# alibaba/TorchEasyRec

Measured on NVIDIA H100. Metric: samples/sec (DLRM-Criteo synth, train step fwd+bwd+optimizer), higher is better.
Workload: dtype f32

## Files before the change

### torcheasyrec_b200/csrc/tzk_interact_wide.cu

```cuda
#include <stdint.h>
#include <stdio.h>
#include <stdlib.h>

#ifdef TZK_CPU_SHIM
#include "cuda_cpu_shim.h"
#include "sm90_cpu_emu.h"
#include "sm90_wgmma_emu.h"
typedef void* tzk_stream_t;
#define TZK_REQUIRE(cond, ...) do { if (!(cond)) return 1; } while (0)
#define TZK_CHECK_LAUNCH(name) do {} while (0)
#else
#include <cuda.h>
#include "tzk_common.cuh"
#define TZK_DYN_SMEM(type, name) extern __shared__ __align__(1024) type name[]
#define TZK_UNPAREN(...) __VA_ARGS__
#define TZK_LAUNCH(kernel, grid, block, smem, stream, ...) TZK_UNPAREN kernel<<<grid, block, smem, stream>>>(__VA_ARGS__)
#endif

namespace {
#ifndef TZK_CPU_SHIM
#include "tzk_sm90_ptx.h"
#endif
#include "tzk_tma.h"
#include "tzk_wgmma.cuh"
namespace tzk_itc {
__device__ __forceinline__ uint32_t cvt_tf32(float x) { return tf32_bits(x); }
__device__ __forceinline__ void mma_tf32(float (&c)[4], const uint32_t (&a)[4], const uint32_t (&b)[2]) { ::mma_tf32(c, a, b); }
}
#include "tzk_interact_tc.cuh"

__device__ __forceinline__ float4 load_l2(const float* p) {
#ifdef TZK_CPU_SHIM
  return *reinterpret_cast<const float4*>(p);
#else
  return __ldcg(reinterpret_cast<const float4*>(p));
#endif
}

constexpr int FB_M = 64;
constexpr int FB_THREADS = 512;
constexpr int FB_WARPS = FB_THREADS / 32;
constexpr int FB_CHUNKS = (tzk_itc::kRow + 31) / 32;
constexpr int FB_PAIR_CHUNKS = tzk_itc::kInter / 32;
constexpr int FB_BOX = 32 * 128;
constexpr int FB_STAGE = 4 * FB_BOX;
constexpr int FB_STAGES = 3;
constexpr int FB_LDP = 360;
constexpr int FB_P_OFF = FB_STAGES * FB_STAGE;
constexpr int FB_S_OFF = FB_P_OFF + FB_M * FB_LDP * 4;
constexpr int FB_IJ_OFF = FB_S_OFF + FB_WARPS * 32 * tzk_itc::kSS * 4;
constexpr int FB_BAR_OFF = FB_IJ_OFF + tzk_itc::kInter * 2;
constexpr int FB_SMEM = FB_BAR_OFF + FB_STAGES * 8;

struct FbParams {
  const float* dz; int64_t ld_dz;
  const float* dense; int64_t ld_dense;
  const float* sparse; int64_t ld_sparse;
  float* d_dense; int64_t ld_ddense;
  float* d_sparse; int64_t ld_dsparse;
  int64_t M;
};

__global__ void __launch_bounds__(FB_THREADS, 1)
interact_wide_bwd_kernel(const __grid_constant__ CUtensorMap map_whi, const __grid_constant__ CUtensorMap map_wlo,
                         FbParams p) {
  TZK_DYN_SMEM(uint8_t, smem);
  float* P = reinterpret_cast<float*>(smem + FB_P_OFF);
  uint64_t* full = reinterpret_cast<uint64_t*>(smem + FB_BAR_OFF);
  const int warp = threadIdx.x >> 5, lane = threadIdx.x & 31, g = lane >> 2, t = lane & 3;
  const int64_t m0 = (int64_t)blockIdx.x * FB_M;

  if (threadIdx.x == 0) {
    for (int s = 0; s < FB_STAGES; ++s) mbar_init(full + s, 1);
    fence_mbarrier_init();
  }
  float* S = reinterpret_cast<float*>(smem + FB_S_OFF) + warp * (32 * tzk_itc::kSS);
  unsigned short* pair_ij = reinterpret_cast<unsigned short*>(smem + FB_IJ_OFF);
  tzk_itc::init_pair_ij(pair_ij);
  for (int i = lane; i < 32 * tzk_itc::kSS; i += 32) S[i] = 0.f;
  __syncthreads();
  auto col_chunk = [](int c) { return (c + FB_PAIR_CHUNKS) % FB_CHUNKS; };
  auto load = [&](int c) {
    uint8_t* sb = smem + (c % FB_STAGES) * FB_STAGE;
    uint64_t* bar = full + c % FB_STAGES;
    const int n0 = col_chunk(c) * 32;
    mbar_expect_tx(bar, FB_STAGE);
    tma_load_2d(sb, &map_whi, bar, 0, n0);
    tma_load_2d(sb + FB_BOX, &map_whi, bar, 32, n0);
    tma_load_2d(sb + 2 * FB_BOX, &map_wlo, bar, 0, n0);
    tma_load_2d(sb + 3 * FB_BOX, &map_wlo, bar, 32, n0);
  };
  if (threadIdx.x == 0)
    for (int c = 0; c < FB_STAGES; ++c) load(c);

  const int wm = warp & 3, wn = warp >> 2;
  const int r = wm * 16 + g;
  uint32_t ah[8][4], al[8][4];
#pragma unroll
  for (int kk = 0; kk < 8; ++kk) {
    const int k0 = kk * 8 + t, k1 = k0 + 4;
    const int64_t ra = m0 + r, rb = ra + 8;
    const float a[4] = {ra < p.M ? __ldg(p.dz + ra * p.ld_dz + k0) : 0.f, rb < p.M ? __ldg(p.dz + rb * p.ld_dz + k0) : 0.f,
                        ra < p.M ? __ldg(p.dz + ra * p.ld_dz + k1) : 0.f, rb < p.M ? __ldg(p.dz + rb * p.ld_dz + k1) : 0.f};
#pragma unroll
    for (int i = 0; i < 4; ++i) {
      ah[kk][i] = tf32_bits(a[i]);
      al[kk][i] = tf32_bits(a[i] - __uint_as_float(ah[kk][i]));
    }
  }
  const int n = wn * 8 + g;
  for (int c = 0; c < FB_CHUNKS; ++c) {
    const int s = c % FB_STAGES;
    mbar_wait(full + s, (uint32_t)(c / FB_STAGES) & 1u);
    const uint32_t* whi = reinterpret_cast<const uint32_t*>(smem + s * FB_STAGE);
    const uint32_t* wlo = whi + 2 * FB_BOX / 4;
    float acc[4] = {0.f, 0.f, 0.f, 0.f};
#pragma unroll
    for (int kk = 0; kk < 8; ++kk) {
      const uint32_t* bh_box = whi + (kk >> 2) * (FB_BOX / 4);
      const uint32_t* bl_box = wlo + (kk >> 2) * (FB_BOX / 4);
      const int k0 = (kk & 3) * 8 + t, k1 = k0 + 4;
      const uint32_t bh[2] = {bh_box[swz(n, k0)], bh_box[swz(n, k1)]};
      const uint32_t bl[2] = {bl_box[swz(n, k0)], bl_box[swz(n, k1)]};
      float part[4] = {0.f, 0.f, 0.f, 0.f};
      mma_tf32(part, al[kk], bh);
      mma_tf32(part, ah[kk], bl);
      mma_tf32(part, ah[kk], bh);
#pragma unroll
      for (int q = 0; q < 4; ++q) acc[q] += part[q];
    }
    const int col = col_chunk(c) * 32 + wn * 8 + 2 * t;
    if (col < tzk_itc::kInter) {
      *reinterpret_cast<float2*>(P + r * FB_LDP + col) = make_float2(acc[0], acc[1]);
      *reinterpret_cast<float2*>(P + (r + 8) * FB_LDP + col) = make_float2(acc[2], acc[3]);
    } else if (col < tzk_itc::kRow) {
      const int e = col - tzk_itc::kInter;
#pragma unroll
      for (int h = 0; h < 2; ++h) {
        const int64_t row = m0 + r + 8 * h;
        if (row >= p.M) continue;
        float* dst = e < tzk_itc::kD ? p.d_dense + row * p.ld_ddense + e : p.d_sparse + row * p.ld_dsparse + (e - tzk_itc::kD);
        *reinterpret_cast<float2*>(dst) = make_float2(acc[2 * h], acc[2 * h + 1]);
      }
    }
    __syncthreads();
    if (threadIdx.x == 0 && c + FB_STAGES < FB_CHUNKS) load(c + FB_STAGES);
  }

  for (int i = warp; i < FB_M; i += FB_WARPS) {
    const int64_t b = m0 + i;
    if (b >= p.M) break;
    float* dd = p.d_dense + b * p.ld_ddense;
    float* ds = p.d_sparse + b * p.ld_dsparse;
    float4 pass[4];
#pragma unroll
    for (int q = 0; q < 4; ++q) {
      const int row = g + 8 * q;
      pass[q] = row == 0 ? load_l2(dd + 4 * t)
              : row < tzk_itc::kN ? load_l2(ds + (row - 1) * tzk_itc::kD + 4 * t)
              : make_float4(0.f, 0.f, 0.f, 0.f);
    }
    tzk_itc::bwd_sample(P + i * FB_LDP, p.dense + b * p.ld_dense, p.sparse + b * p.ld_sparse, pass, pair_ij, S, dd, ds,
                        lane);
  }
}

constexpr int FF_M = 128;
constexpr int FF_THREADS = 256;
constexpr int FF_WARPS = FF_THREADS / 32;
constexpr int FF_X_BYTES = FF_M * 128;
constexpr int FF_W_BYTES = 64 * 128;
constexpr int FF_STAGE = FF_X_BYTES + 2 * FF_W_BYTES;
constexpr int FF_STAGES = 3;
constexpr int FF_E_OFF = FF_STAGES * FF_STAGE;
constexpr int FF_BAR_OFF = FF_E_OFF + FF_X_BYTES;
constexpr int FF_SMEM = FF_BAR_OFF + FF_STAGES * 8;
static_assert(FF_WARPS * tzk_itc::kInter * 4 <= FF_X_BYTES, "staging rows overflow their region");
constexpr int FF_SPARSE0 = tzk_itc::kInter + tzk_itc::kD;

struct FfParams {
  const float* dense; int64_t ld_dense;
  const float* sparse; int64_t ld_sparse;
  float* pairs; int64_t ld_pairs;
  const float* bias;
  float* y; int64_t ld_y;
  int64_t M;
};

__device__ __forceinline__ void fence_proxy_async() {
#ifndef TZK_CPU_SHIM
  asm volatile("fence.proxy.async;" ::: "memory");
#endif
}

__global__ void __launch_bounds__(FF_THREADS, 2)
interact_wide_fwd_kernel(const __grid_constant__ CUtensorMap map_pairs, const __grid_constant__ CUtensorMap map_dense,
                         const __grid_constant__ CUtensorMap map_sparse, const __grid_constant__ CUtensorMap map_whi, const __grid_constant__ CUtensorMap map_wlo,
                         FfParams p) {
  TZK_DYN_SMEM(uint8_t, smem);
  uint64_t* full = reinterpret_cast<uint64_t*>(smem + FF_BAR_OFF);
  const int warp = threadIdx.x >> 5, lane = threadIdx.x & 31, g = lane >> 2, t = lane & 3;
  const int64_t m0 = (int64_t)blockIdx.x * FF_M;
  const int64_t m_end = p.M - m0 < FF_M ? p.M : m0 + FF_M;

  if (threadIdx.x == 0) {
    for (int s = 0; s < FF_STAGES; ++s) mbar_init(full + s, 1);
    fence_mbarrier_init();
  }
  {
    float* O = reinterpret_cast<float*>(smem + FF_E_OFF) + warp * tzk_itc::kInter;
    if (lane == 0) O[tzk_itc::kP] = 0.f;
    int rowbase[4];
    tzk_itc::pair_rowbase(g, rowbase);
    int64_t b = m0 + warp;
    float4 x[4];
    if (b < m_end) {
#pragma unroll
      for (int j = 0; j < 4; ++j) x[j] = tzk_itc::load_x4(p.dense + b * p.ld_dense, p.sparse + b * p.ld_sparse, g + 8 * j, 4 * t);
    }
    for (; b < m_end; b += FF_WARPS) {
      float4 xn[4];
      const int64_t bn = b + FF_WARPS;
      if (bn < m_end) {
#pragma unroll
        for (int j = 0; j < 4; ++j)
          xn[j] = tzk_itc::load_x4(p.dense + bn * p.ld_dense, p.sparse + bn * p.ld_sparse, g + 8 * j, 4 * t);
      }
      tzk_itc::fwd_sample(x, rowbase, O, p.pairs + b * p.ld_pairs, lane);
      if (bn < m_end) {
#pragma unroll
        for (int j = 0; j < 4; ++j) x[j] = xn[j];
      }
    }
  }
  fence_proxy_async();
  __syncthreads();

  auto load = [&](int c) {
    uint8_t* sb = smem + (c % FF_STAGES) * FF_STAGE;
    uint64_t* bar = full + c % FF_STAGES;
    mbar_expect_tx(bar, c == FB_PAIR_CHUNKS ? FF_STAGE + FF_X_BYTES : FF_STAGE);
    if (c < FB_PAIR_CHUNKS) {
      tma_load_2d(sb, &map_pairs, bar, 32 * c, (int)m0);
    } else if (c == FB_PAIR_CHUNKS) {
      tma_load_2d(sb, &map_dense, bar, 0, (int)m0);
      tma_load_2d(smem + FF_E_OFF, &map_sparse, bar, 0, (int)m0);
    } else {
      tma_load_2d(sb, &map_sparse, bar, 32 * c - FF_SPARSE0, (int)m0);
    }
    tma_load_2d(sb + FF_X_BYTES, &map_whi, bar, 32 * c, 0);
    tma_load_2d(sb + FF_X_BYTES + FF_W_BYTES, &map_wlo, bar, 32 * c, 0);
  };
  if (threadIdx.x == 0)
    for (int c = 0; c < FF_STAGES; ++c) load(c);

  const int r = warp * 16 + g;
  float acc[32], part[32];
#pragma unroll
  for (int i = 0; i < 32; ++i) acc[i] = 0.f;
  for (int c = 0; c < FB_CHUNKS; ++c) {
    const int s = c % FF_STAGES;
    mbar_wait(full + s, (uint32_t)(c / FF_STAGES) & 1u);
    const float* xs = reinterpret_cast<const float*>(smem + s * FF_STAGE);
    const uint8_t* whi = smem + s * FF_STAGE + FF_X_BYTES;
    const uint8_t* wlo = whi + FF_W_BYTES;
#pragma unroll
    for (int ks = 0; ks < 4; ++ks) {
      const int k0 = ks * 8 + t, k1 = k0 + 4;
      const bool sp = ks >= 2 && c == FB_PAIR_CHUNKS;
      const float* as = sp ? reinterpret_cast<const float*>(smem + FF_E_OFF) : xs;
      const int x16 = sp ? 16 : 0;
      const float a[4] = {as[swz(r, k0) ^ x16], as[swz(r + 8, k0) ^ x16], as[swz(r, k1) ^ x16], as[swz(r + 8, k1) ^ x16]};
      uint32_t ah[4], al[4];
#pragma unroll
      for (int i = 0; i < 4; ++i) {
        ah[i] = tf32_bits(a[i]);
        al[i] = tf32_bits(a[i] - __uint_as_float(ah[i]));
      }
      wgmma_fence();
      wgmma_3xtf32<64>(part, ah, al, wgmma_desc(whi, ks), wgmma_desc(wlo, ks));
      wgmma_commit();
      wgmma_wait<0>();
#pragma unroll
      for (int i = 0; i < 32; ++i) {
        wgmma_reg_fence(part[i]);
        acc[i] += part[i];
      }
    }
    __syncthreads();
    if (threadIdx.x == 0 && c + FF_STAGES < FB_CHUNKS) load(c + FF_STAGES);
  }
#pragma unroll
  for (int nt = 0; nt < 8; ++nt) {
    const int col = nt * 8 + 2 * t;
    const float b0 = p.bias ? __ldg(p.bias + col) : 0.f, b1 = p.bias ? __ldg(p.bias + col + 1) : 0.f;
#pragma unroll
    for (int h = 0; h < 2; ++h) {
      const int64_t row = m0 + r + 8 * h;
      if (row >= p.M) continue;
      float2 o = make_float2(acc[4 * nt + 2 * h] + b0, acc[4 * nt + 2 * h + 1] + b1);
      o.x = fmaxf(o.x, 0.f);
      o.y = fmaxf(o.y, 0.f);
      *reinterpret_cast<float2*>(p.y + row * p.ld_y + col) = o;
    }
  }
}

__global__ void split_w_kernel(const float* __restrict__ w, int64_t ld_w, int K, float* __restrict__ hi,
                               float* __restrict__ lo) {
  const int i = blockIdx.x * blockDim.x + threadIdx.x;
  if (i < K * 64) {
    const float v = w[(int64_t)(i / K) * ld_w + i % K];
    const float h = tf32_rna(v);
    hi[i] = h;
    lo[i] = tf32_rna(v - h);
  }
}

#include "tzk_wgrad3x.cuh"

constexpr int WW_ZT = 64 * 128;

__global__ void __launch_bounds__(WG_THREADS, 2)
interact_wide_wgrad_kernel(const __grid_constant__ CUtensorMap map_x0, const __grid_constant__ CUtensorMap map_x1,
                           const __grid_constant__ CUtensorMap map_x2, const __grid_constant__ CUtensorMap map_dz,
                           WgParams p) {
  TZK_DYN_SMEM(uint8_t, smem);
  uint8_t* zt = smem + WG_STAGES * WG_STAGE;
  uint64_t* full = reinterpret_cast<uint64_t*>(zt + 2 * WW_ZT);
  int* boxes = reinterpret_cast<int*>(full + WG_STAGES);

  const int warp = threadIdx.x >> 5, lane = threadIdx.x & 31, g = lane >> 2, t = lane & 3;
  const int jt = blockIdx.x % p.k_tiles;
  const int64_t slab = blockIdx.x / p.k_tiles;
  const int64_t row0 = slab * p.slab_rows;
  const int64_t rows = (p.M - row0 < p.slab_rows) ? p.M - row0 : p.slab_rows;
  const int num_c = (int)((rows + WG_ROWS - 1) / WG_ROWS);

  if (threadIdx.x == 0) {
    for (int s = 0; s < WG_STAGES; ++s) mbar_init(full + s, 1);
    fence_mbarrier_init();
    for (int b = 0; b < 4; ++b) {
      const int box = jt * 4 + b, s = wg_source(p.src, box);
      boxes[b] = s;
      boxes[4 + b] = wg_pick(p.src.col0, s) + 32 * (box - wg_pick(p.src.first, s));
    }
  }
  __syncthreads();
  auto load = [&](int c) {
    uint8_t* sb = smem + (c % WG_STAGES) * WG_STAGE;
    uint64_t* bar = full + c % WG_STAGES;
    const int r = (int)(row0 + (int64_t)c * WG_ROWS);
    mbar_expect_tx(bar, WG_A + WG_B);
#pragma unroll 1
    for (int b = 0; b < 4; ++b) {
      const int s = *reinterpret_cast<volatile int*>(boxes + b), col = *reinterpret_cast<volatile int*>(boxes + 4 + b);
      tma_load_2d(sb + b * WG_BOX, s == 0 ? &map_x0 : s == 1 ? &map_x1 : &map_x2, bar, col, r);
    }
#pragma unroll
    for (int b = 0; b < 2; ++b) tma_load_2d(sb + WG_A + b * WG_BOX, &map_dz, bar, b * 32, r);
  };
  if (threadIdx.x == 0)
    for (int c = 0; c < WG_STAGES && c < num_c; ++c) load(c);

  const int xc = (warp >> 2) * 64 + (warp & 3) * 16 + g;
  const int tn = threadIdx.x & 63, tq = threadIdx.x >> 6;
  uint32_t* zhi = reinterpret_cast<uint32_t*>(zt);
  uint32_t* zlo = zhi + WW_ZT / 4;
  float acc[32], part[32];
#pragma unroll
  for (int i = 0; i < 32; ++i) acc[i] = 0.f;
  for (int c = 0; c < num_c; ++c) {
    const int s = c % WG_STAGES;
    mbar_wait(full + s, (uint32_t)(c / WG_STAGES) & 1u);
    const float* xs = reinterpret_cast<const float*>(smem + s * WG_STAGE);
    const float* zs = reinterpret_cast<const float*>(smem + s * WG_STAGE + WG_A);
    auto at = [](const float* base, int m, int col) { return base[(col >> 5) * (WG_BOX / 4) + swz(m, col & 31)]; };
#pragma unroll
    for (int h = 0; h < 2; ++h) {
      const int m = 4 * tq + 16 * h;
      float hi[4], lo[4];
#pragma unroll
      for (int j = 0; j < 4; ++j) {
        const float v = at(zs, m + j, tn);
        hi[j] = tf32_rna(v);
        lo[j] = tf32_rna(v - hi[j]);
      }
      *reinterpret_cast<float4*>(zhi + swz(tn, m)) = make_float4(hi[0], hi[1], hi[2], hi[3]);
      *reinterpret_cast<float4*>(zlo + swz(tn, m)) = make_float4(lo[0], lo[1], lo[2], lo[3]);
    }
    fence_proxy_async();
    __syncthreads();
#pragma unroll
    for (int ks = 0; ks < WG_ROWS / 8; ++ks) {
      const int m = ks * 8 + t;
      const float a[4] = {at(xs, m, xc), at(xs, m, xc + 8), at(xs, m + 4, xc), at(xs, m + 4, xc + 8)};
      uint32_t ah[4], al[4];
#pragma unroll
      for (int i = 0; i < 4; ++i) {
        ah[i] = tf32_bits(a[i]);
        al[i] = tf32_bits(a[i] - __uint_as_float(ah[i]));
      }
      wgmma_fence();
      wgmma_tf32<64>(part, ah, wgmma_desc(zlo, ks), false);
      wgmma_tf32<64>(part, al, wgmma_desc(zhi, ks), true);
      wgmma_tf32<64>(part, ah, wgmma_desc(zhi, ks), true);
      wgmma_commit();
      wgmma_wait<0>();
#pragma unroll
      for (int i = 0; i < 32; ++i) {
        wgmma_reg_fence(part[i]);
        acc[i] += part[i];
      }
    }
    __syncthreads();
    if (threadIdx.x == 0 && c + WG_STAGES < num_c) load(c + WG_STAGES);
  }
  float* out = p.partial + ((int64_t)slab * p.k_tiles + jt) * 128 * 64;
#pragma unroll
  for (int i = 0; i < 8; ++i)
#pragma unroll
    for (int h = 0; h < 2; ++h)
      *reinterpret_cast<float2*>(out + (int64_t)(xc + 8 * h) * 64 + 8 * i + 2 * t) =
          make_float2(acc[4 * i + 2 * h], acc[4 * i + 2 * h + 1]);
}

__global__ void split_wt_kernel(const float* __restrict__ w, int64_t ld_w, int K, float* __restrict__ hi,
                                float* __restrict__ lo) {
  const int i = blockIdx.x * blockDim.x + threadIdx.x;
  if (i < K * 64) {
    const int k = i >> 6, o = i & 63;
    const float v = w[(int64_t)o * ld_w + k];
    const float h = tf32_rna(v);
    hi[i] = h;
    lo[i] = tf32_rna(v - h);
  }
}

}

extern "C" int tzk_interact_wide_bwd(const float* dz, int64_t ld_dz, const float* w, int64_t ld_w, const float* dense,
                                     int64_t ld_dense, const float* sparse, int64_t ld_sparse, int64_t M, float* d_dense,
                                     int64_t ld_ddense, float* d_sparse, int64_t ld_dsparse, float* wt_hi, float* wt_lo,
                                     tzk_stream_t stream) {
  TZK_REQUIRE(M > 0, "interact_wide_bwd: M must be positive");
  TZK_REQUIRE(ld_w >= tzk_itc::kRow, "interact_wide_bwd: w needs %d columns", tzk_itc::kRow);
  const int64_t lds[] = {ld_dz, ld_w, ld_dense, ld_sparse, ld_ddense, ld_dsparse};
  for (int64_t ld : lds) TZK_REQUIRE(ld % 4 == 0, "interact_wide_bwd: row strides must be multiples of 4 floats");
  const void* ptrs[] = {dz, w, dense, sparse, d_dense, d_sparse, wt_hi, wt_lo};
  for (const void* q : ptrs)
    TZK_REQUIRE(q && reinterpret_cast<uintptr_t>(q) % 16 == 0, "interact_wide_bwd: NULL or not 16-B aligned pointer");
  cudaStream_t st = reinterpret_cast<cudaStream_t>(stream);
  TZK_LAUNCH((split_wt_kernel), (tzk_itc::kRow * 64 + 255) / 256, 256, 0, st, w, ld_w, tzk_itc::kRow, wt_hi, wt_lo);
  CUtensorMap mh, ml;
  TZK_REQUIRE(!make_map(&mh, wt_hi, tzk_itc::kRow, 64, 64, 32) && !make_map(&ml, wt_lo, tzk_itc::kRow, 64, 64, 32),
              "interact_wide_bwd: tensor-map encoding failed");
  FbParams p;
  p.dz = dz; p.ld_dz = ld_dz; p.dense = dense; p.ld_dense = ld_dense; p.sparse = sparse; p.ld_sparse = ld_sparse;
  p.d_dense = d_dense; p.ld_ddense = ld_ddense; p.d_sparse = d_sparse; p.ld_dsparse = ld_dsparse; p.M = M;
#ifndef TZK_CPU_SHIM
  static bool configured = false;
  if (!configured) {
    cudaFuncSetAttribute(interact_wide_bwd_kernel, cudaFuncAttributeMaxDynamicSharedMemorySize, FB_SMEM);
    configured = true;
  }
#endif
  TZK_LAUNCH((interact_wide_bwd_kernel), (unsigned)((M + FB_M - 1) / FB_M), FB_THREADS, FB_SMEM, st, mh, ml, p);
  TZK_CHECK_LAUNCH("interact_wide_bwd_kernel");
  return 0;
}

extern "C" int tzk_interact_wide_fwd(const float* dense, int64_t ld_dense, const float* sparse, int64_t ld_sparse,
                                     const float* w, int64_t ld_w, const float* bias, int64_t M, float* y, int64_t ld_y,
                                     float* pairs, int64_t ld_pairs, float* w_hi, float* w_lo, tzk_stream_t stream) {
  TZK_REQUIRE(M > 0, "interact_wide_fwd: M must be positive");
  TZK_REQUIRE(ld_w >= tzk_itc::kRow && ld_y >= 64 && ld_pairs >= tzk_itc::kInter && ld_dense >= tzk_itc::kD &&
              ld_sparse >= tzk_itc::kRow - FF_SPARSE0, "interact_wide_fwd: row stride shorter than the row");
  const int64_t lds[] = {ld_dense, ld_sparse, ld_w, ld_y, ld_pairs};
  for (int64_t ld : lds) TZK_REQUIRE(ld % 4 == 0, "interact_wide_fwd: row strides must be multiples of 4 floats");
  const void* ptrs[] = {dense, sparse, w, y, pairs, w_hi, w_lo};
  for (const void* q : ptrs)
    TZK_REQUIRE(q && reinterpret_cast<uintptr_t>(q) % 16 == 0, "interact_wide_fwd: NULL or not 16-B aligned pointer");
  cudaStream_t st = reinterpret_cast<cudaStream_t>(stream);
  TZK_LAUNCH((split_w_kernel), (tzk_itc::kRow * 64 + 255) / 256, 256, 0, st, w, ld_w, tzk_itc::kRow, w_hi, w_lo);
  CUtensorMap mp, md, ms, mh, ml;
  TZK_REQUIRE(!make_map(&mp, pairs, M, tzk_itc::kInter, ld_pairs, FF_M) &&
              !make_map(&md, dense, M, tzk_itc::kD, ld_dense, FF_M) &&
              !make_map(&ms, sparse, M, tzk_itc::kRow - FF_SPARSE0, ld_sparse, FF_M) &&
              !make_map(&mh, w_hi, 64, tzk_itc::kRow, tzk_itc::kRow, 64) &&
              !make_map(&ml, w_lo, 64, tzk_itc::kRow, tzk_itc::kRow, 64), "interact_wide_fwd: tensor-map encoding failed");
  FfParams p;
  p.dense = dense; p.ld_dense = ld_dense; p.sparse = sparse; p.ld_sparse = ld_sparse; p.pairs = pairs;
  p.ld_pairs = ld_pairs; p.bias = bias; p.y = y; p.ld_y = ld_y; p.M = M;
#ifndef TZK_CPU_SHIM
  static bool configured = false;
  if (!configured) {
    cudaFuncSetAttribute(interact_wide_fwd_kernel, cudaFuncAttributeMaxDynamicSharedMemorySize, FF_SMEM);
    configured = true;
  }
#endif
  TZK_LAUNCH((interact_wide_fwd_kernel), (unsigned)((M + FF_M - 1) / FF_M), FF_THREADS, FF_SMEM, st, mp, md, ms, mh, ml, p);
  TZK_CHECK_LAUNCH("interact_wide_fwd_kernel");
  return 0;
}

extern "C" int tzk_interact_wide_wgrad(const float* dz, int64_t ld_dz, const float* pairs, int64_t ld_pairs,
                                       const float* dense, int64_t ld_dense, const float* sparse, int64_t ld_sparse,
                                       int64_t M, int32_t slabs, float* partial, float* dw, int64_t ld_dw,
                                       tzk_stream_t stream) {
  TZK_REQUIRE(M > 0 && slabs > 0, "interact_wide_wgrad: M and slabs must be positive");
  TZK_REQUIRE(ld_dw >= tzk_itc::kRow, "interact_wide_wgrad: dw needs %d columns", tzk_itc::kRow);
  const int64_t lds[] = {ld_dz, ld_pairs, ld_dense, ld_sparse};
  for (int64_t ld : lds) TZK_REQUIRE(ld % 4 == 0, "interact_wide_wgrad: row strides must be multiples of 4 floats");
  const void* ptrs[] = {dz, pairs, dense, sparse, partial, dw};
  for (const void* q : ptrs)
    TZK_REQUIRE(q && reinterpret_cast<uintptr_t>(q) % 16 == 0, "interact_wide_wgrad: NULL or not 16-B aligned pointer");
  CUtensorMap mx[WG_SRC], mz;
  TZK_REQUIRE(!make_map(&mx[0], pairs, M, tzk_itc::kInter, ld_pairs, WG_ROWS) &&
              !make_map(&mx[1], sparse, M, tzk_itc::kRow - FF_SPARSE0, ld_sparse, WG_ROWS) &&
              !make_map(&mx[2], dense, M, tzk_itc::kD, ld_dense, WG_ROWS) &&
              !make_map(&mz, dz, M, 64, ld_dz, WG_ROWS), "interact_wide_wgrad: tensor-map encoding failed");
  const WgSources src = {{0, FB_PAIR_CHUNKS, FB_CHUNKS - 1, FB_CHUNKS}, {0, 0, 0}, {0, FF_SPARSE0, tzk_itc::kInter},
                         {tzk_itc::kInter, tzk_itc::kRow - FF_SPARSE0, tzk_itc::kD}};
  TZK_REQUIRE(wgrad3x_launch<interact_wide_wgrad_kernel>(mx, mz, src, M, slabs, partial, dw, ld_dw,
                                                         reinterpret_cast<cudaStream_t>(stream), 2 * WW_ZT) == 0,
              "interact_wide_wgrad: launch failed");
  return 0;
}
```

### torcheasyrec_b200/csrc/tzk_sm90_ptx.h

```cpp

__device__ __forceinline__ uint32_t smem_u32(const void* p) { return (uint32_t)__cvta_generic_to_shared(p); }

__device__ __forceinline__ void mbar_init(uint64_t* bar, uint32_t count) {
  asm volatile("mbarrier.init.shared::cta.b64 [%0], %1;" ::"r"(smem_u32(bar)), "r"(count));
}
__device__ __forceinline__ void mbar_expect_tx(uint64_t* bar, uint32_t bytes) {
  asm volatile("mbarrier.arrive.expect_tx.shared::cta.b64 _, [%0], %1;" ::"r"(smem_u32(bar)), "r"(bytes) : "memory");
}
__device__ __forceinline__ void mbar_wait(uint64_t* bar, uint32_t parity) {
  asm volatile(
      "{\n\t.reg .pred p;\n\t"
      "WAIT_LOOP:\n\t"
      "mbarrier.try_wait.parity.shared::cta.b64 p, [%0], %1;\n\t"
      "@p bra DONE;\n\t"
      "bra WAIT_LOOP;\n\t"
      "DONE:\n\t}" ::"r"(smem_u32(bar)), "r"(parity)
      : "memory");
}
__device__ __forceinline__ void fence_mbarrier_init() { asm volatile("fence.mbarrier_init.release.cluster;" ::: "memory"); }

__device__ __forceinline__ void tma_load_2d(void* dst, const CUtensorMap* map, uint64_t* bar, int c0, int c1) {
  asm volatile(
      "cp.async.bulk.tensor.2d.shared::cluster.global.mbarrier::complete_tx::bytes [%0], [%1, {%3, %4}], [%2];"
      ::"r"(smem_u32(dst)), "l"(map), "r"(smem_u32(bar)), "r"(c0), "r"(c1)
      : "memory");
}

__device__ __forceinline__ uint32_t tf32_bits(float x) {
  uint32_t r;
  asm("cvt.rna.tf32.f32 %0, %1;" : "=r"(r) : "f"(x));
  return r;
}
__device__ __forceinline__ float tf32_rna(float x) { return __uint_as_float(tf32_bits(x)); }
__device__ __forceinline__ void mma_tf32(float (&c)[4], const uint32_t (&a)[4], const uint32_t (&b)[2]) {
  asm volatile("mma.sync.aligned.m16n8k8.row.col.f32.tf32.tf32.f32 {%0,%1,%2,%3}, {%4,%5,%6,%7}, {%8,%9}, {%0,%1,%2,%3};"
               : "+f"(c[0]), "+f"(c[1]), "+f"(c[2]), "+f"(c[3])
               : "r"(a[0]), "r"(a[1]), "r"(a[2]), "r"(a[3]), "r"(b[0]), "r"(b[1]));
}
```

### torcheasyrec_b200/csrc/tzk_wgmma.cuh

```cuda
#pragma once

__device__ __forceinline__ uint64_t wgmma_desc(const void* box, int ks) {
  const uint32_t a = smem_u32(box) + 32u * (uint32_t)ks;
  return (uint64_t)((a >> 4) & 0x3fffu) | (1ull << 16) | ((uint64_t)(1024 >> 4) << 32) | (1ull << 62);
}

#ifndef TZK_CPU_SHIM
__device__ __forceinline__ void wgmma_fence() { asm volatile("wgmma.fence.sync.aligned;" ::: "memory"); }
__device__ __forceinline__ void wgmma_commit() { asm volatile("wgmma.commit_group.sync.aligned;" ::: "memory"); }
template <int N>
__device__ __forceinline__ void wgmma_wait() { asm volatile("wgmma.wait_group.sync.aligned %0;" ::"n"(N) : "memory"); }
__device__ __forceinline__ void wgmma_reg_fence(float& r) { asm volatile("" : "+f"(r)::"memory"); }

template <int N>
__device__ __forceinline__ void wgmma_tf32(float (&d)[N / 2], const uint32_t (&a)[4], uint64_t desc, bool scale_d);

template <>
__device__ __forceinline__ void wgmma_tf32<64>(float (&d)[32], const uint32_t (&a)[4], uint64_t desc, bool scale_d) {
  asm volatile(
      "{\n\t.reg .pred p;\n\tsetp.ne.b32 p, %37, 0;\n\t"
      "wgmma.mma_async.sync.aligned.m64n64k8.f32.tf32.tf32 "
      "{%0,%1,%2,%3,%4,%5,%6,%7,%8,%9,%10,%11,%12,%13,%14,%15,"
      "%16,%17,%18,%19,%20,%21,%22,%23,%24,%25,%26,%27,%28,%29,%30,%31}, {%32,%33,%34,%35}, %36, p, 1, 1;\n\t}"
      : "+f"(d[0]), "+f"(d[1]), "+f"(d[2]), "+f"(d[3]), "+f"(d[4]), "+f"(d[5]), "+f"(d[6]), "+f"(d[7]),
        "+f"(d[8]), "+f"(d[9]), "+f"(d[10]), "+f"(d[11]), "+f"(d[12]), "+f"(d[13]), "+f"(d[14]), "+f"(d[15]),
        "+f"(d[16]), "+f"(d[17]), "+f"(d[18]), "+f"(d[19]), "+f"(d[20]), "+f"(d[21]), "+f"(d[22]), "+f"(d[23]),
        "+f"(d[24]), "+f"(d[25]), "+f"(d[26]), "+f"(d[27]), "+f"(d[28]), "+f"(d[29]), "+f"(d[30]), "+f"(d[31])
      : "r"(a[0]), "r"(a[1]), "r"(a[2]), "r"(a[3]), "l"(desc), "r"((int)scale_d));
}
#endif

template <int N>
__device__ __forceinline__ void wgmma_3xtf32(float (&part)[N / 2], const uint32_t (&ah)[4], const uint32_t (&al)[4],
                                             uint64_t hi_b, uint64_t lo_b) {
  wgmma_tf32<N>(part, al, hi_b, false);
  wgmma_tf32<N>(part, ah, lo_b, true);
  wgmma_tf32<N>(part, ah, hi_b, true);
}
```

Before: 50.59 million.

## Warp-specialize interaction backward into persistent wgmma producer and per-sample consumer warps

Restructures the interaction backward kernel into a persistent grid sized to the SM count. One warpgroup computes the dz·W GEMM with 3xTF32 wgmma (m64n32) through a 4-stage TMA pipeline with empty/full mbarriers. The other twelve warps run the per-sample backward on the previous tile's P buffer, handing off through p_full/p_free barriers, with L2 prefetch of inputs and setmaxnreg register rebalancing. The aim is to overlap GEMM and per-sample work across tiles instead of serializing them within one block. It adds barrier handshakes and fewer per-sample warps, and the single shared P buffer can stall the GEMM warps while the sample warps catch up.

```diff
diff --git a/torcheasyrec_b200/csrc/tzk_interact_wide.cu b/torcheasyrec_b200/csrc/tzk_interact_wide.cu
--- a/torcheasyrec_b200/csrc/tzk_interact_wide.cu
+++ b/torcheasyrec_b200/csrc/tzk_interact_wide.cu
@@ -5,6 +5,7 @@
 #ifdef TZK_CPU_SHIM
 #include "cuda_cpu_shim.h"
 #include "sm90_cpu_emu.h"
+#include "sm90_arrive_emu.h"
 #include "sm90_wgmma_emu.h"
 typedef void* tzk_stream_t;
 #define TZK_REQUIRE(cond, ...) do { if (!(cond)) return 1; } while (0)
@@ -36,21 +37,36 @@
   return __ldcg(reinterpret_cast<const float4*>(p));
 #endif
 }
+__device__ __forceinline__ void fence_cta() {
+#ifndef TZK_CPU_SHIM
+  __threadfence_block();
+#endif
+}
+__device__ __forceinline__ void prefetch_l2(const float* p) {
+#ifndef TZK_CPU_SHIM
+  asm volatile("prefetch.global.L2 [%0];" ::"l"(p));
+#else
+  (void)p;
+#endif
+}
 
 constexpr int FB_M = 64;
 constexpr int FB_THREADS = 512;
-constexpr int FB_WARPS = FB_THREADS / 32;
+constexpr int FB_SAMPLE_WARPS = FB_THREADS / 32 - 4;
+constexpr int FB_GEMM_REGS = 176, FB_SAMPLE_REGS = 112;
 constexpr int FB_CHUNKS = (tzk_itc::kRow + 31) / 32;
 constexpr int FB_PAIR_CHUNKS = tzk_itc::kInter / 32;
+constexpr int FB_PASS_CHUNKS = FB_CHUNKS - FB_PAIR_CHUNKS;
 constexpr int FB_BOX = 32 * 128;
 constexpr int FB_STAGE = 4 * FB_BOX;
-constexpr int FB_STAGES = 3;
+constexpr int FB_STAGES = 4;
 constexpr int FB_LDP = 360;
 constexpr int FB_P_OFF = FB_STAGES * FB_STAGE;
 constexpr int FB_S_OFF = FB_P_OFF + FB_M * FB_LDP * 4;
-constexpr int FB_IJ_OFF = FB_S_OFF + FB_WARPS * 32 * tzk_itc::kSS * 4;
+constexpr int FB_IJ_OFF = FB_S_OFF + FB_SAMPLE_WARPS * 32 * tzk_itc::kSS * 4;
 constexpr int FB_BAR_OFF = FB_IJ_OFF + tzk_itc::kInter * 2;
-constexpr int FB_SMEM = FB_BAR_OFF + FB_STAGES * 8;
+constexpr int FB_SMEM = FB_BAR_OFF + (2 * FB_STAGES + 2) * 8;
+static_assert(FB_BAR_OFF % 8 == 0 && FB_SMEM <= 232448, "shared-memory layout of interact_wide_bwd_kernel");
 
 struct FbParams {
   const float* dz; int64_t ld_dz;
@@ -67,23 +83,68 @@
   TZK_DYN_SMEM(uint8_t, smem);
   float* P = reinterpret_cast<float*>(smem + FB_P_OFF);
   uint64_t* full = reinterpret_cast<uint64_t*>(smem + FB_BAR_OFF);
+  uint64_t* empty = full + FB_STAGES;
+  uint64_t* p_full = empty + FB_STAGES;
+  uint64_t* p_free = p_full + 1;
   const int warp = threadIdx.x >> 5, lane = threadIdx.x & 31, g = lane >> 2, t = lane & 3;
-  const int64_t m0 = (int64_t)blockIdx.x * FB_M;
+  const int64_t tiles = (p.M + FB_M - 1) / FB_M;
+  const int my_tiles = (int)((tiles - blockIdx.x + gridDim.x - 1) / gridDim.x);
 
   if (threadIdx.x == 0) {
-    for (int s = 0; s < FB_STAGES; ++s) mbar_init(full + s, 1);
+    for (int s = 0; s < FB_STAGES; ++s) {
+      mbar_init(full + s, 1);
+      mbar_init(empty + s, 4);
+    }
+    mbar_init(p_full, 4);
+    mbar_init(p_free, FB_SAMPLE_WARPS);
     fence_mbarrier_init();
   }
-  float* S = reinterpret_cast<float*>(smem + FB_S_OFF) + warp * (32 * tzk_itc::kSS);
   unsigned short* pair_ij = reinterpret_cast<unsigned short*>(smem + FB_IJ_OFF);
   tzk_itc::init_pair_ij(pair_ij);
-  for (int i = lane; i < 32 * tzk_itc::kSS; i += 32) S[i] = 0.f;
   __syncthreads();
+
+  if (warp >= 4) {
+    setmaxnreg_dec<FB_SAMPLE_REGS>();
+    const int sw = warp - 4;
+    float* S = reinterpret_cast<float*>(smem + FB_S_OFF) + sw * (32 * tzk_itc::kSS);
+    for (int i = lane; i < 32 * tzk_itc::kSS; i += 32) S[i] = 0.f;
+    __syncwarp();
+    for (int it = 0; it < my_tiles; ++it) {
+      const int64_t m0 = ((int64_t)blockIdx.x + (int64_t)it * gridDim.x) * FB_M;
+      for (int i = sw; i < FB_M && m0 + i < p.M; i += FB_SAMPLE_WARPS) {
+        if (lane < 13) prefetch_l2(p.sparse + (m0 + i) * p.ld_sparse + 32 * lane);
+        else if (lane == 13) prefetch_l2(p.dense + (m0 + i) * p.ld_dense);
+      }
+      mbar_wait(p_full, (uint32_t)it & 1u);
+      for (int i = sw; i < FB_M; i += FB_SAMPLE_WARPS) {
+        const int64_t b = m0 + i;
+        if (b >= p.M) break;
+        float* dd = p.d_dense + b * p.ld_ddense;
+        float* ds = p.d_sparse + b * p.ld_dsparse;
+        float4 pass[4];
+#pragma unroll
+        for (int q = 0; q < 4; ++q) {
+          const int row = g + 8 * q;
+          pass[q] = row == 0 ? load_l2(dd + 4 * t)
+                  : row < tzk_itc::kN ? load_l2(ds + (row - 1) * tzk_itc::kD + 4 * t)
+                  : make_float4(0.f, 0.f, 0.f, 0.f);
+        }
+        tzk_itc::bwd_sample(P + i * FB_LDP, p.dense + b * p.ld_dense, p.sparse + b * p.ld_sparse, pass, pair_ij, S, dd,
+                            ds, lane);
+      }
+      __syncwarp();
+      if (lane == 0) mbar_arrive(p_free);
+    }
+    return;
+  }
+
+  setmaxnreg_inc<FB_GEMM_REGS>();
+  const int total = my_tiles * FB_CHUNKS;
   auto col_chunk = [](int c) { return (c + FB_PAIR_CHUNKS) % FB_CHUNKS; };
-  auto load = [&](int c) {
-    uint8_t* sb = smem + (c % FB_STAGES) * FB_STAGE;
-    uint64_t* bar = full + c % FB_STAGES;
-    const int n0 = col_chunk(c) * 32;
+  auto load = [&](int q) {
+    uint8_t* sb = smem + (q % FB_STAGES) * FB_STAGE;
+    uint64_t* bar = full + q % FB_STAGES;
+    const int n0 = col_chunk(q % FB_CHUNKS) * 32;
     mbar_expect_tx(bar, FB_STAGE);
     tma_load_2d(sb, &map_whi, bar, 0, n0);
     tma_load_2d(sb + FB_BOX, &map_whi, bar, 32, n0);
@@ -91,77 +152,96 @@
     tma_load_2d(sb + 3 * FB_BOX, &map_wlo, bar, 32, n0);
   };
   if (threadIdx.x == 0)
-    for (int c = 0; c < FB_STAGES; ++c) load(c);
-
-  const int wm = warp & 3, wn = warp >> 2;
-  const int r = wm * 16 + g;
-  uint32_t ah[8][4], al[8][4];
-#pragma unroll
-  for (int kk = 0; kk < 8; ++kk) {
-    const int k0 = kk * 8 + t, k1 = k0 + 4;
+    for (int q = 0; q < FB_STAGES; ++q) load(q);
+
+  const int r = warp * 16 + g;
+  float a[8][4];
+  auto load_dz = [&](int64_t m0) {
     const int64_t ra = m0 + r, rb = ra + 8;
-    const float a[4] = {ra < p.M ? __ldg(p.dz + ra * p.ld_dz + k0) : 0.f, rb < p.M ? __ldg(p.dz + rb * p.ld_dz + k0) : 0.f,
-                        ra < p.M ? __ldg(p.dz + ra * p.ld_dz + k1) : 0.f, rb < p.M ? __ldg(p.dz + rb * p.ld_dz + k1) : 0.f};
-#pragma unroll
-    for (int i = 0; i < 4; ++i) {
-      ah[kk][i] = tf32_bits(a[i]);
-      al[kk][i] = tf32_bits(a[i] - __uint_as_float(ah[kk][i]));
-    }
-  }
-  const int n = wn * 8 + g;
-  for (int c = 0; c < FB_CHUNKS; ++c) {
-    const int s = c % FB_STAGES;
-    mbar_wait(full + s, (uint32_t)(c / FB_STAGES) & 1u);
-    const uint32_t* whi = reinterpret_cast<const uint32_t*>(smem + s * FB_STAGE);
-    const uint32_t* wlo = whi + 2 * FB_BOX / 4;
-    float acc[4] = {0.f, 0.f, 0.f, 0.f};
 #pragma unroll
     for (int kk = 0; kk < 8; ++kk) {
-      const uint32_t* bh_box = whi + (kk >> 2) * (FB_BOX / 4);
-      const uint32_t* bl_box = wlo + (kk >> 2) * (FB_BOX / 4);
-      const int k0 = (kk & 3) * 8 + t, k1 = k0 + 4;
-      const uint32_t bh[2] = {bh_box[swz(n, k0)], bh_box[swz(n, k1)]};
-      const uint32_t bl[2] = {bl_box[swz(n, k0)], bl_box[swz(n, k1)]};
-      float part[4] = {0.f, 0.f, 0.f, 0.f};
-      mma_tf32(part, al[kk], bh);
-      mma_tf32(part, ah[kk], bl);
-      mma_tf32(part, ah[kk], bh);
-#pragma unroll
-      for (int q = 0; q < 4; ++q) acc[q] += part[q];
-    }
-    const int col = col_chunk(c) * 32 + wn * 8 + 2 * t;
-    if (col < tzk_itc::kInter) {
-      *reinterpret_cast<float2*>(P + r * FB_LDP + col) = make_float2(acc[0], acc[1]);
-      *reinterpret_cast<float2*>(P + (r + 8) * FB_LDP + col) = make_float2(acc[2], acc[3]);
-    } else if (col < tzk_itc::kRow) {
-      const int e = col - tzk_itc::kInter;
-#pragma unroll
-      for (int h = 0; h < 2; ++h) {
-        const int64_t row = m0 + r + 8 * h;
-        if (row >= p.M) continue;
-        float* dst = e < tzk_itc::kD ? p.d_dense + row * p.ld_ddense + e : p.d_sparse + row * p.ld_dsparse + (e - tzk_itc::kD);
-        *reinterpret_cast<float2*>(dst) = make_float2(acc[2 * h], acc[2 * h + 1]);
-      }
-    }
-    __syncthreads();
-    if (threadIdx.x == 0 && c + FB_STAGES < FB_CHUNKS) load(c + FB_STAGES);
-  }
-
-  for (int i = warp; i < FB_M; i += FB_WARPS) {
-    const int64_t b = m0 + i;
-    if (b >= p.M) break;
-    float* dd = p.d_dense + b * p.ld_ddense;
-    float* ds = p.d_sparse + b * p.ld_dsparse;
-    float4 pass[4];
-#pragma unroll
-    for (int q = 0; q < 4; ++q) {
-      const int row = g + 8 * q;
-      pass[q] = row == 0 ? load_l2(dd + 4 * t)
-              : row < tzk_itc::kN ? load_l2(ds + (row - 1) * tzk_itc::kD + 4 * t)
-              : make_float4(0.f, 0.f, 0.f, 0.f);
-    }
-    tzk_itc::bwd_sample(P + i * FB_LDP, p.dense + b * p.ld_dense, p.sparse + b * p.ld_sparse, pass, pair_ij, S, dd, ds,
-                        lane);
+      const int k0 = kk * 8 + t, k1 = k0 + 4;
+      a[kk][0] = ra < p.M ? __ldg(p.dz + ra * p.ld_dz + k0) : 0.f;
+      a[kk][1] = rb < p.M ? __ldg(p.dz + rb * p.ld_dz + k0) : 0.f;
+      a[kk][2] = ra < p.M ? __ldg(p.dz + ra * p.ld_dz + k1) : 0.f;
+      a[kk][3] = rb < p.M ? __ldg(p.dz + rb * p.ld_dz + k1) : 0.f;
+    }
+  };
+  load_dz((int64_t)blockIdx.x * FB_M);
+  int q = 0;
+  for (int it = 0; it < my_tiles; ++it) {
+    const int64_t m0 = ((int64_t)blockIdx.x + (int64_t)it * gridDim.x) * FB_M;
+    uint32_t ah[8][4], al[8][4];
+#pragma unroll
+    for (int kk = 0; kk < 8; ++kk)
+#pragma unroll
+      for (int i = 0; i < 4; ++i) {
+        ah[kk][i] = tf32_bits(a[kk][i]);
+        al[kk][i] = tf32_bits(a[kk][i] - __uint_as_float(ah[kk][i]));
+      }
+    if (it + 1 < my_tiles) load_dz(m0 + (int64_t)gridDim.x * FB_M);
+    for (int c = 0; c < FB_CHUNKS; ++c, ++q) {
+      if (threadIdx.x == 0 && q > 0 && q - 1 + FB_STAGES < total) {
+        mbar_wait(empty + (q - 1) % FB_STAGES, (uint32_t)((q - 1) / FB_STAGES) & 1u);
+        load(q - 1 + FB_STAGES);
+      }
+      if (c == FB_PASS_CHUNKS && it > 0) mbar_wait(p_free, (uint32_t)(it - 1) & 1u);
+      const int s = q % FB_STAGES;
+      mbar_wait(full + s, (uint32_t)(q / FB_STAGES) & 1u);
+      const uint8_t* whi = smem + s * FB_STAGE;
+      const uint8_t* wlo = whi + 2 * FB_BOX;
+      float acc[16], part[2][16];
+#pragma unroll
+      for (int i = 0; i < 16; ++i) acc[i] = 0.f;
+      wgmma_fence();
+      wgmma_3xtf32<32>(part[0], ah[0], al[0], wgmma_desc(whi, 0), wgmma_desc(wlo, 0));
+      wgmma_commit();
+#pragma unroll
+      for (int kk = 0; kk < 8; ++kk) {
+        if (kk + 1 < 8) {
+          const int kn = kk + 1;
+          wgmma_fence();
+          wgmma_3xtf32<32>(part[kn & 1], ah[kn], al[kn], wgmma_desc(whi + (kn >> 2) * FB_BOX, kn & 3),
+                           wgmma_desc(wlo + (kn >> 2) * FB_BOX, kn & 3));
+          wgmma_commit();
+          wgmma_wait<1>();
+        } else {
+          wgmma_wait<0>();
+        }
+#pragma unroll
+        for (int i = 0; i < 16; ++i) {
+          wgmma_reg_fence(part[kk & 1][i]);
+          acc[i] += part[kk & 1][i];
+        }
+      }
+      __syncwarp();
+      if (lane == 0) mbar_arrive(empty + s);
+      const int col0 = col_chunk(c) * 32 + 2 * t;
+      if (c >= FB_PASS_CHUNKS) {
+#pragma unroll
+        for (int i = 0; i < 4; ++i) {
+          *reinterpret_cast<float2*>(P + r * FB_LDP + col0 + 8 * i) = make_float2(acc[4 * i], acc[4 * i + 1]);
+          *reinterpret_cast<float2*>(P + (r + 8) * FB_LDP + col0 + 8 * i) = make_float2(acc[4 * i + 2], acc[4 * i + 3]);
+        }
+      } else {
+#pragma unroll
+        for (int i = 0; i < 4; ++i) {
+          const int col = col0 + 8 * i;
+          if (col >= tzk_itc::kRow) continue;
+          const int e = col - tzk_itc::kInter;
+#pragma unroll
+          for (int h = 0; h < 2; ++h) {
+            const int64_t row = m0 + r + 8 * h;
+            if (row >= p.M) continue;
+            float* dst = e < tzk_itc::kD ? p.d_dense + row * p.ld_ddense + e : p.d_sparse + row * p.ld_dsparse + (e - tzk_itc::kD);
+            *reinterpret_cast<float2*>(dst) = make_float2(acc[4 * i + 2 * h], acc[4 * i + 2 * h + 1]);
+          }
+        }
+      }
+    }
+    fence_cta();
+    __syncwarp();
+    if (lane == 0) mbar_arrive(p_full);
   }
 }
 
@@ -439,10 +519,10 @@
 
 }
 
-extern "C" int tzk_interact_wide_bwd(const float* dz, int64_t ld_dz, const float* w, int64_t ld_w, const float* dense,
-                                     int64_t ld_dense, const float* sparse, int64_t ld_sparse, int64_t M, float* d_dense,
-                                     int64_t ld_ddense, float* d_sparse, int64_t ld_dsparse, float* wt_hi, float* wt_lo,
-                                     tzk_stream_t stream) {
+static int interact_wide_bwd_launch(const float* dz, int64_t ld_dz, const float* w, int64_t ld_w, const float* dense,
+                                    int64_t ld_dense, const float* sparse, int64_t ld_sparse, int64_t M, float* d_dense,
+                                    int64_t ld_ddense, float* d_sparse, int64_t ld_dsparse, float* wt_hi, float* wt_lo,
+                                    int max_ctas, tzk_stream_t stream) {
   TZK_REQUIRE(M > 0, "interact_wide_bwd: M must be positive");
   TZK_REQUIRE(ld_w >= tzk_itc::kRow, "interact_wide_bwd: w needs %d columns", tzk_itc::kRow);
   const int64_t lds[] = {ld_dz, ld_w, ld_dense, ld_sparse, ld_ddense, ld_dsparse};
@@ -459,16 +539,46 @@
   p.dz = dz; p.ld_dz = ld_dz; p.dense = dense; p.ld_dense = ld_dense; p.sparse = sparse; p.ld_sparse = ld_sparse;
   p.d_dense = d_dense; p.ld_ddense = ld_ddense; p.d_sparse = d_sparse; p.ld_dsparse = ld_dsparse; p.M = M;
 #ifndef TZK_CPU_SHIM
-  static bool configured = false;
-  if (!configured) {
+  static int sms = 0;
+  if (!sms) {
+    int dev = 0;
+    TZK_REQUIRE(cudaGetDevice(&dev) == cudaSuccess &&
+                cudaDeviceGetAttribute(&sms, cudaDevAttrMultiProcessorCount, dev) == cudaSuccess && sms > 0,
+                "interact_wide_bwd: cannot read the SM count");
     cudaFuncSetAttribute(interact_wide_bwd_kernel, cudaFuncAttributeMaxDynamicSharedMemorySize, FB_SMEM);
-    configured = true;
-  }
-#endif
-  TZK_LAUNCH((interact_wide_bwd_kernel), (unsigned)((M + FB_M - 1) / FB_M), FB_THREADS, FB_SMEM, st, mh, ml, p);
+  }
+  if (!max_ctas) max_ctas = sms;
+#endif
+  const int64_t tiles = (M + FB_M - 1) / FB_M;
+  TZK_LAUNCH((interact_wide_bwd_kernel), (unsigned)(tiles < max_ctas ? tiles : max_ctas), FB_THREADS, FB_SMEM, st, mh, ml,
+             p);
   TZK_CHECK_LAUNCH("interact_wide_bwd_kernel");
   return 0;
 }
+
+extern "C" int tzk_interact_wide_bwd(const float* dz, int64_t ld_dz, const float* w, int64_t ld_w, const float* dense,
+                                     int64_t ld_dense, const float* sparse, int64_t ld_sparse, int64_t M, float* d_dense,
+                                     int64_t ld_ddense, float* d_sparse, int64_t ld_dsparse, float* wt_hi, float* wt_lo,
+                                     tzk_stream_t stream) {
+#ifdef TZK_CPU_SHIM
+  const int max_ctas = 132;
+#else
+  const int max_ctas = 0;
+#endif
+  return interact_wide_bwd_launch(dz, ld_dz, w, ld_w, dense, ld_dense, sparse, ld_sparse, M, d_dense, ld_ddense, d_sparse,
+                                  ld_dsparse, wt_hi, wt_lo, max_ctas, stream);
+}
+
+#ifdef TZK_CPU_SHIM
+extern "C" int tzk_interact_wide_bwd_ctas(const float* dz, int64_t ld_dz, const float* w, int64_t ld_w, const float* dense,
+                                          int64_t ld_dense, const float* sparse, int64_t ld_sparse, int64_t M,
+                                          float* d_dense, int64_t ld_ddense, float* d_sparse, int64_t ld_dsparse,
+                                          float* wt_hi, float* wt_lo, int32_t ctas) {
+  if (ctas <= 0) return 1;
+  return interact_wide_bwd_launch(dz, ld_dz, w, ld_w, dense, ld_dense, sparse, ld_sparse, M, d_dense, ld_ddense, d_sparse,
+                                  ld_dsparse, wt_hi, wt_lo, ctas, nullptr);
+}
+#endif
 
 extern "C" int tzk_interact_wide_fwd(const float* dense, int64_t ld_dense, const float* sparse, int64_t ld_sparse,
                                      const float* w, int64_t ld_w, const float* bias, int64_t M, float* y, int64_t ld_y,
diff --git a/torcheasyrec_b200/csrc/tzk_sm90_ptx.h b/torcheasyrec_b200/csrc/tzk_sm90_ptx.h
--- a/torcheasyrec_b200/csrc/tzk_sm90_ptx.h
+++ b/torcheasyrec_b200/csrc/tzk_sm90_ptx.h
@@ -6,6 +6,9 @@
 }
 __device__ __forceinline__ void mbar_expect_tx(uint64_t* bar, uint32_t bytes) {
   asm volatile("mbarrier.arrive.expect_tx.shared::cta.b64 _, [%0], %1;" ::"r"(smem_u32(bar)), "r"(bytes) : "memory");
+}
+__device__ __forceinline__ void mbar_arrive(uint64_t* bar) {
+  asm volatile("mbarrier.arrive.shared::cta.b64 _, [%0];" ::"r"(smem_u32(bar)) : "memory");
 }
 __device__ __forceinline__ void mbar_wait(uint64_t* bar, uint32_t parity) {
   asm volatile(
@@ -18,6 +21,11 @@
       : "memory");
 }
 __device__ __forceinline__ void fence_mbarrier_init() { asm volatile("fence.mbarrier_init.release.cluster;" ::: "memory"); }
+
+template <int N>
+__device__ __forceinline__ void setmaxnreg_inc() { asm volatile("setmaxnreg.inc.sync.aligned.u32 %0;" ::"n"(N)); }
+template <int N>
+__device__ __forceinline__ void setmaxnreg_dec() { asm volatile("setmaxnreg.dec.sync.aligned.u32 %0;" ::"n"(N)); }
 
 __device__ __forceinline__ void tma_load_2d(void* dst, const CUtensorMap* map, uint64_t* bar, int c0, int c1) {
   asm volatile(
diff --git a/torcheasyrec_b200/csrc/tzk_wgmma.cuh b/torcheasyrec_b200/csrc/tzk_wgmma.cuh
--- a/torcheasyrec_b200/csrc/tzk_wgmma.cuh
+++ b/torcheasyrec_b200/csrc/tzk_wgmma.cuh
@@ -14,6 +14,17 @@
 
 template <int N>
 __device__ __forceinline__ void wgmma_tf32(float (&d)[N / 2], const uint32_t (&a)[4], uint64_t desc, bool scale_d);
+
+template <>
+__device__ __forceinline__ void wgmma_tf32<32>(float (&d)[16], const uint32_t (&a)[4], uint64_t desc, bool scale_d) {
+  asm volatile(
+      "{\n\t.reg .pred p;\n\tsetp.ne.b32 p, %21, 0;\n\t"
+      "wgmma.mma_async.sync.aligned.m64n32k8.f32.tf32.tf32 "
+      "{%0,%1,%2,%3,%4,%5,%6,%7,%8,%9,%10,%11,%12,%13,%14,%15}, {%16,%17,%18,%19}, %20, p, 1, 1;\n\t}"
+      : "+f"(d[0]), "+f"(d[1]), "+f"(d[2]), "+f"(d[3]), "+f"(d[4]), "+f"(d[5]), "+f"(d[6]), "+f"(d[7]),
+        "+f"(d[8]), "+f"(d[9]), "+f"(d[10]), "+f"(d[11]), "+f"(d[12]), "+f"(d[13]), "+f"(d[14]), "+f"(d[15])
+      : "r"(a[0]), "r"(a[1]), "r"(a[2]), "r"(a[3]), "l"(desc), "r"((int)scale_d));
+}
 
 template <>
 __device__ __forceinline__ void wgmma_tf32<64>(float (&d)[32], const uint32_t (&a)[4], uint64_t desc, bool scale_d) {
```

Result: faster. 51.80 million (median of 6 runs) (+2.4%).

## Use per-warpgroup wgmma m64n32 for wide interaction backward GEMM

Applied to the files above, without the earlier changes.

Replaces the per-warp mma.sync 3xTF32 GEMM in the wide interaction backward kernel with warpgroup wgmma m64n32k8. Each of the four warpgroups now handles its own 32-column chunk per round, so one round covers four chunks. The TMA ring is regrouped into two stages of four chunks each, and the per-warp S scratch tiles now reuse the ring's shared memory after the GEMM loop, keeping total shared memory in bounds. Each k-step waits on its wgmma before accumulating, which serialises issue. Register fragments of dz are reused as wgmma A operands, which assumes their layout matches the wgmma A-fragment layout.

```diff
diff --git a/torcheasyrec_b200/csrc/tzk_interact_wide.cu b/torcheasyrec_b200/csrc/tzk_interact_wide.cu
--- a/torcheasyrec_b200/csrc/tzk_interact_wide.cu
+++ b/torcheasyrec_b200/csrc/tzk_interact_wide.cu
@@ -40,17 +40,21 @@
 constexpr int FB_M = 64;
 constexpr int FB_THREADS = 512;
 constexpr int FB_WARPS = FB_THREADS / 32;
+constexpr int FB_WGS = FB_WARPS / 4;
 constexpr int FB_CHUNKS = (tzk_itc::kRow + 31) / 32;
 constexpr int FB_PAIR_CHUNKS = tzk_itc::kInter / 32;
+constexpr int FB_ROUNDS = (FB_CHUNKS + FB_WGS - 1) / FB_WGS;
 constexpr int FB_BOX = 32 * 128;
-constexpr int FB_STAGE = 4 * FB_BOX;
-constexpr int FB_STAGES = 3;
+constexpr int FB_CHUNK = 4 * FB_BOX;
+constexpr int FB_STAGE = FB_WGS * FB_CHUNK;
+constexpr int FB_STAGES = 2;
 constexpr int FB_LDP = 360;
+constexpr int FB_S_OFF = 0;
 constexpr int FB_P_OFF = FB_STAGES * FB_STAGE;
-constexpr int FB_S_OFF = FB_P_OFF + FB_M * FB_LDP * 4;
-constexpr int FB_IJ_OFF = FB_S_OFF + FB_WARPS * 32 * tzk_itc::kSS * 4;
+constexpr int FB_IJ_OFF = FB_P_OFF + FB_M * FB_LDP * 4;
 constexpr int FB_BAR_OFF = FB_IJ_OFF + tzk_itc::kInter * 2;
 constexpr int FB_SMEM = FB_BAR_OFF + FB_STAGES * 8;
+static_assert(FB_S_OFF + FB_WARPS * 32 * tzk_itc::kSS * 4 <= FB_P_OFF, "the S tiles overflow the ring");
 
 struct FbParams {
   const float* dz; int64_t ld_dz;
@@ -74,26 +78,28 @@
     for (int s = 0; s < FB_STAGES; ++s) mbar_init(full + s, 1);
     fence_mbarrier_init();
   }
-  float* S = reinterpret_cast<float*>(smem + FB_S_OFF) + warp * (32 * tzk_itc::kSS);
   unsigned short* pair_ij = reinterpret_cast<unsigned short*>(smem + FB_IJ_OFF);
   tzk_itc::init_pair_ij(pair_ij);
-  for (int i = lane; i < 32 * tzk_itc::kSS; i += 32) S[i] = 0.f;
   __syncthreads();
   auto col_chunk = [](int c) { return (c + FB_PAIR_CHUNKS) % FB_CHUNKS; };
-  auto load = [&](int c) {
-    uint8_t* sb = smem + (c % FB_STAGES) * FB_STAGE;
-    uint64_t* bar = full + c % FB_STAGES;
-    const int n0 = col_chunk(c) * 32;
-    mbar_expect_tx(bar, FB_STAGE);
-    tma_load_2d(sb, &map_whi, bar, 0, n0);
-    tma_load_2d(sb + FB_BOX, &map_whi, bar, 32, n0);
-    tma_load_2d(sb + 2 * FB_BOX, &map_wlo, bar, 0, n0);
-    tma_load_2d(sb + 3 * FB_BOX, &map_wlo, bar, 32, n0);
+  auto load = [&](int j) {
+    uint8_t* sb = smem + (j % FB_STAGES) * FB_STAGE;
+    uint64_t* bar = full + j % FB_STAGES;
+    const int nc = FB_CHUNKS - FB_WGS * j < FB_WGS ? FB_CHUNKS - FB_WGS * j : FB_WGS;
+    mbar_expect_tx(bar, nc * FB_CHUNK);
+    for (int w = 0; w < nc; ++w) {
+      uint8_t* cb = sb + w * FB_CHUNK;
+      const int n0 = col_chunk(FB_WGS * j + w) * 32;
+      tma_load_2d(cb, &map_whi, bar, 0, n0);
+      tma_load_2d(cb + FB_BOX, &map_whi, bar, 32, n0);
+      tma_load_2d(cb + 2 * FB_BOX, &map_wlo, bar, 0, n0);
+      tma_load_2d(cb + 3 * FB_BOX, &map_wlo, bar, 32, n0);
+    }
   };
   if (threadIdx.x == 0)
-    for (int c = 0; c < FB_STAGES; ++c) load(c);
-
-  const int wm = warp & 3, wn = warp >> 2;
+    for (int j = 0; j < FB_STAGES; ++j) load(j);
+
+  const int wm = warp & 3, wg = warp >> 2;
   const int r = wm * 16 + g;
   uint32_t ah[8][4], al[8][4];
 #pragma unroll
@@ -108,45 +114,54 @@
       al[kk][i] = tf32_bits(a[i] - __uint_as_float(ah[kk][i]));
     }
   }
-  const int n = wn * 8 + g;
-  for (int c = 0; c < FB_CHUNKS; ++c) {
-    const int s = c % FB_STAGES;
-    mbar_wait(full + s, (uint32_t)(c / FB_STAGES) & 1u);
-    const uint32_t* whi = reinterpret_cast<const uint32_t*>(smem + s * FB_STAGE);
-    const uint32_t* wlo = whi + 2 * FB_BOX / 4;
-    float acc[4] = {0.f, 0.f, 0.f, 0.f};
-#pragma unroll
-    for (int kk = 0; kk < 8; ++kk) {
-      const uint32_t* bh_box = whi + (kk >> 2) * (FB_BOX / 4);
-      const uint32_t* bl_box = wlo + (kk >> 2) * (FB_BOX / 4);
-      const int k0 = (kk & 3) * 8 + t, k1 = k0 + 4;
-      const uint32_t bh[2] = {bh_box[swz(n, k0)], bh_box[swz(n, k1)]};
-      const uint32_t bl[2] = {bl_box[swz(n, k0)], bl_box[swz(n, k1)]};
-      float part[4] = {0.f, 0.f, 0.f, 0.f};
-      mma_tf32(part, al[kk], bh);
-      mma_tf32(part, ah[kk], bl);
-      mma_tf32(part, ah[kk], bh);
-#pragma unroll
-      for (int q = 0; q < 4; ++q) acc[q] += part[q];
-    }
-    const int col = col_chunk(c) * 32 + wn * 8 + 2 * t;
-    if (col < tzk_itc::kInter) {
-      *reinterpret_cast<float2*>(P + r * FB_LDP + col) = make_float2(acc[0], acc[1]);
-      *reinterpret_cast<float2*>(P + (r + 8) * FB_LDP + col) = make_float2(acc[2], acc[3]);
-    } else if (col < tzk_itc::kRow) {
-      const int e = col - tzk_itc::kInter;
-#pragma unroll
-      for (int h = 0; h < 2; ++h) {
-        const int64_t row = m0 + r + 8 * h;
-        if (row >= p.M) continue;
-        float* dst = e < tzk_itc::kD ? p.d_dense + row * p.ld_ddense + e : p.d_sparse + row * p.ld_dsparse + (e - tzk_itc::kD);
-        *reinterpret_cast<float2*>(dst) = make_float2(acc[2 * h], acc[2 * h + 1]);
+  for (int j = 0; j < FB_ROUNDS; ++j) {
+    const int s = j % FB_STAGES, c = FB_WGS * j + wg;
+    mbar_wait(full + s, (uint32_t)(j / FB_STAGES) & 1u);
+    if (c < FB_CHUNKS) {
+      const uint8_t* whi = smem + s * FB_STAGE + wg * FB_CHUNK;
+      const uint8_t* wlo = whi + 2 * FB_BOX;
+      float acc[16], part[16];
+#pragma unroll
+      for (int i = 0; i < 16; ++i) acc[i] = 0.f;
+#pragma unroll
+      for (int kk = 0; kk < 8; ++kk) {
+        const int box = (kk >> 2) * FB_BOX, ks = kk & 3;
+        wgmma_fence();
+        wgmma_3xtf32<32>(part, ah[kk], al[kk], wgmma_desc(whi + box, ks), wgmma_desc(wlo + box, ks));
+        wgmma_commit();
+        wgmma_wait<0>();
+#pragma unroll
+        for (int i = 0; i < 16; ++i) {
+          wgmma_reg_fence(part[i]);
+          acc[i] += part[i];
+        }
+      }
+#pragma unroll
+      for (int nt = 0; nt < 4; ++nt) {
+        const int col = col_chunk(c) * 32 + nt * 8 + 2 * t;
+        if (col < tzk_itc::kInter) {
+          *reinterpret_cast<float2*>(P + r * FB_LDP + col) = make_float2(acc[4 * nt], acc[4 * nt + 1]);
+          *reinterpret_cast<float2*>(P + (r + 8) * FB_LDP + col) = make_float2(acc[4 * nt + 2], acc[4 * nt + 3]);
+        } else if (col < tzk_itc::kRow) {
+          const int e = col - tzk_itc::kInter;
+#pragma unroll
+          for (int h = 0; h < 2; ++h) {
+            const int64_t row = m0 + r + 8 * h;
+            if (row >= p.M) continue;
+            float* dst = e < tzk_itc::kD ? p.d_dense + row * p.ld_ddense + e
+                                         : p.d_sparse + row * p.ld_dsparse + (e - tzk_itc::kD);
+            *reinterpret_cast<float2*>(dst) = make_float2(acc[4 * nt + 2 * h], acc[4 * nt + 2 * h + 1]);
+          }
+        }
       }
     }
     __syncthreads();
-    if (threadIdx.x == 0 && c + FB_STAGES < FB_CHUNKS) load(c + FB_STAGES);
-  }
-
+    if (threadIdx.x == 0 && j + FB_STAGES < FB_ROUNDS) load(j + FB_STAGES);
+  }
+
+  float* S = reinterpret_cast<float*>(smem + FB_S_OFF) + warp * (32 * tzk_itc::kSS);
+  for (int i = lane; i < 32 * tzk_itc::kSS; i += 32) S[i] = 0.f;
+  __syncwarp();
   for (int i = warp; i < FB_M; i += FB_WARPS) {
     const int64_t b = m0 + i;
     if (b >= p.M) break;
diff --git a/torcheasyrec_b200/csrc/tzk_wgmma.cuh b/torcheasyrec_b200/csrc/tzk_wgmma.cuh
--- a/torcheasyrec_b200/csrc/tzk_wgmma.cuh
+++ b/torcheasyrec_b200/csrc/tzk_wgmma.cuh
@@ -28,6 +28,17 @@
         "+f"(d[24]), "+f"(d[25]), "+f"(d[26]), "+f"(d[27]), "+f"(d[28]), "+f"(d[29]), "+f"(d[30]), "+f"(d[31])
       : "r"(a[0]), "r"(a[1]), "r"(a[2]), "r"(a[3]), "l"(desc), "r"((int)scale_d));
 }
+
+template <>
+__device__ __forceinline__ void wgmma_tf32<32>(float (&d)[16], const uint32_t (&a)[4], uint64_t desc, bool scale_d) {
+  asm volatile(
+      "{\n\t.reg .pred p;\n\tsetp.ne.b32 p, %21, 0;\n\t"
+      "wgmma.mma_async.sync.aligned.m64n32k8.f32.tf32.tf32 "
+      "{%0,%1,%2,%3,%4,%5,%6,%7,%8,%9,%10,%11,%12,%13,%14,%15}, {%16,%17,%18,%19}, %20, p, 1, 1;\n\t}"
+      : "+f"(d[0]), "+f"(d[1]), "+f"(d[2]), "+f"(d[3]), "+f"(d[4]), "+f"(d[5]), "+f"(d[6]), "+f"(d[7]),
+        "+f"(d[8]), "+f"(d[9]), "+f"(d[10]), "+f"(d[11]), "+f"(d[12]), "+f"(d[13]), "+f"(d[14]), "+f"(d[15])
+      : "r"(a[0]), "r"(a[1]), "r"(a[2]), "r"(a[3]), "l"(desc), "r"((int)scale_d));
+}
 #endif
 
 template <int N>
```

New measurement: 50.74 million before, 52.85 million after, median of 6. 4.2% higher.
